# bridgedp/hunter_bipedal_control

Measured on AMD Instinct MI355X. Metric: MPC+WBC updates/sec (batch=4096, N=100, 12-DoF), higher is better.
Workload: dtype f64; 1 GPU; 4096 distinct hunter instances (4096/GPU, state seed 1234 + id), trot gait from t = 0.1, cmd_vel (0.3, 0, 0, 0), N=100 shooting intervals (dt 0.015 s), node tables generated on the device (hb_refgen_update, per-knot IK joint references), 1 SQP iteration + WeightedWbc per update, x0 of every call perturbed by measurement noise (sigma 0.01) so that no call re-solves a converged problem: every line s; batch_per_gpu=4096, total_instances=4096, horizon_nodes=100

## Files before the change

### hunter_bipedal_control_amd/csrc/hb_lq.hpp

```cpp
#pragma once
#include "hb_model.hpp"
#include "hb_tile.hpp"

namespace hb {

struct DevConfig {
  double Q_diag[HB_NX];
  double R_FF_diag[12];
  double R_jj[HB_NJ * HB_NJ];
  double friction_mu, friction_reg, friction_gripper, friction_shift, fb_mu, fb_delta;
  double soft_w;
  double pos_b[2], vel_b[2], force_b[2], force_lim[2];
  double kp_normal, zv_gain, zv_off, xy_gain;
  double g_max, g_min, alpha_decay, alpha_min, gamma_c, armijo, delta_tol;
  double torque_limits[5];
  double wbc_mu, swing_kp, swing_kd, bh_kp, bh_kd, ba_kp, ba_kd, w_swing, w_base, w_force, wbc_eps;
  int wbc_max_iter, wbc_type;
  double default_joint_state[HB_NJ];
  int debug_stop;
  int wbc_reg_steps;
  int wbc_eps_mode;
};

constexpr int NU_T = 12;
// ... 417 lines not shown
      const int s_n = c_slot(i, 0), s_x = c_slot(i, 1);
      CDt[r * 12 + s_n] = cf[i] ? v[3 * i + 2] : v[3 * i];
      CDt[r * 12 + s_x] = cf[i] ? v[3 * i] : v[3 * i + 1];
      CDt[r * 12 + s_x + 1] = cf[i] ? v[3 * i + 1] : v[3 * i + 2];
    }
  }
  {
    const double inv_m = rcp_t(M.total_mass);
    WaveTile<2, 1> tl;
    tile_init(cx, tl, 29, 9, [J2](int r, int c) {
      const double v = J2[((r >= 19 ? r : 19) - 10) * 9 + c];
      return r >= 19 ? v : 0.0;
    });
    tile_mma<8, 9, false, 9, false, 6>(cx, tl, J1, J2 + 27, 29, 9);
    tile_store_pre(cx, tl, 29, 9, [J1, J2](int r, int c) { return J1[r * 9 + c] + J2[r * 9 + c]; },
                   [ABt, dt](int r, int c, double acc, double j12) {
                     const int dir = j_dir(r), i = j_frow(c);
                     ABt[dir * 12 + i] = (dir == i ? 1.0 : 0.0) + 0.5 * dt * j12 + 0.5 * dt * dt * acc;
                   });
    for (int idx = cx.lane; idx < 108 + 132 + 27; idx += cx.nlanes) {
      if (idx < 108) {
        const int fd = idx / 9, c = idx - 9 * fd, j = fd / 3, a = fd - 3 * j;
        double g1[3], g2[3];
#pragma unroll
        for (int pt = 0; pt < 2; ++pt) {
          const double* fr_in = lds + LqLds::fr_slot(pt, j);
          const double rx = fr_in[0], ry = fr_in[1], rz = fr_in[2];
          double* g = pt == 0 ? g1 : g2;
          g[0] = (a == 1 ? -rz : (a == 2 ? ry : 0.0)) * inv_m;
          g[1] = (a == 0 ? rz : (a == 2 ? -rx : 0.0)) * inv_m;
          g[2] = (a == 0 ? -ry : (a == 1 ? rx : 0.0)) * inv_m;
        }
        double acc = inv_m * J2[a * 9 + c];
#pragma unroll
        for (int k = 0; k < 3; ++k) acc += J2[(3 + k) * 9 + c] * g1[k];
        const double lin = c < 3 ? g1[c] + g2[c] : 0.0;
        ABt[(22 + fd) * 12 + j_frow(c)] = 0.5 * dt * lin + 0.5 * dt * dt * acc;
      } else if (idx < 240) {
        const int e = idx - 108, dir = e / 3, i = e - 3 * dir;
        const bool force_i = dir >= 22 && dir < 34 && (dir - 22) % 3 == i;
        ABt[dir * 12 + i] = (dir == i ? 1.0 : 0.0) + (force_i ? dt * inv_m : 0.0);
      } else {
        const int e = idx - 240, dir = 6 + e / 9, i = 3 + e % 9;
        ABt[dir * 12 + i] = dir == i ? 1.0 : 0.0;
      }
    }
  }
  for (int i = cx.lane; i < 22; i += cx.nlanes)
    xplus[i] = (i < 12) ? xs[i] + 0.5 * dt * (fv[i] + xplus[i]) : xs[i] + dt * us[i];
  cx.sync();
#if defined(__HIP_DEVICE_COMPILE__)
  if (cx.lane < 22) { lds[LqLds::park + cx.lane] = xref_reg; lds[LqLds::xnext_park + cx.lane] = xnext_reg; }
#endif
  HB_ABLATE_STOP(C.debug_stop == form::LQ_COMPOSE);
  int n_f = 0;
  for (int i = 0; i < HB_NC; ++i)
    if (cf[i]) n_f += 3;

  {
    WaveTile<1, 2> tg;
    tile_init(cx, tg, 10, 32, [](int, int) { return 0.0; });
    tile_mma<12, 12, false, 12, true>(cx, tg, CDt + 22 * 12, CDt, 10, 32, [cfm](int slot) { return slot_is_eq(slot, cfm) ? 1.0 : 0.0; },
                                      EqStepLive{cfm});
    tile_store(cx, tg, 10, 32, [W, GtG](int k, int r, double v) {
      double* dst = r < 22 ? W + k * 23 + r : GtG + k * 10 + r - 22;
      *dst = v;
    });
  }
  for (int k = cx.lane; k < 10; k += cx.nlanes) {
    double s = 0;
#pragma unroll
    for (int slot = 0; slot < 12; ++slot) {
      const double w = slot_is_eq(slot, cfm) ? 1.0 : 0.0;
      s += (w * CDt[(22 + k) * 12 + slot]) * rowval[slot];
    }
    W[k * 23 + 22] = s;
  }
  cx.sync();
  double* Lc = Kx;
  double* col = Kx + 100;
  double* Linv = Kx + 112;
  int rank_l = 0, donemask = 0;
  int ei0 = 0, ej0 = cx.lane;
  while (ej0 > ei0) { ej0 -= ei0 + 1; ++ei0; }
#if defined(__HIP_DEVICE_COMPILE__)
  {
    static_assert(Ctx::nlanes == 64, "one triangle element per lane");
    const bool own = cx.lane < 55;
    const bool diag = own && ei0 == ej0;
    double g = own ? GtG[ei0 * 10 + ej0] : 0.0;
    const double tol = 1e-10 * wave_max_pos_f64(diag ? g : 0.0);
    for (int i = cx.lane; i < 124; i += cx.nlanes) Kx[i] = 0.0;
    cx.sync();
    for (int st = 0; st < 10; ++st) {
      const double v = (diag && !((donemask >> ei0) & 1)) ? g : -1.0;
      const double best = wave_max_pos_f64(v);
      if (!(best > tol)) break;
      const unsigned long long hit = __ballot(v == best);
      const int ps = __builtin_amdgcn_readlane(ei0, __ffsll(hit) - 1);
      const double rinv = rsqrt_t(best), lss = best * rinv;
      if (own && (ei0 == ps || ej0 == ps)) {
        const int k = (ei0 == ps) ? ej0 : ei0;
        if (!((donemask >> k) & 1)) {
          const double l = (k == ps) ? lss : g * rinv;
          col[k] = l;
          Lc[st * 10 + k] = l;
        }
      }
      if (cx.lane == 0) { perm[st] = ps; Linv[st] = rinv; }
      cx.sync();
      donemask |= 1 << ps;
      if (own && !((donemask >> ei0) & 1) && !((donemask >> ej0) & 1)) g -= col[ei0] * col[ej0];
      cx.sync();
      rank_l = st + 1;
    }
  }
#else
  double tol;
  {
    double dmax0 = 0;
    for (int i = 0; i < 10; ++i) dmax0 = fmax(dmax0, GtG[i * 10 + i]);
    tol = 1e-10 * dmax0;
  }
  for (int i = cx.lane; i < 124; i += cx.nlanes) Kx[i] = 0.0;
  cx.sync();
  for (int st = 0; st < 10; ++st) {
    int ps = -1;
    double best = -1.0;
    for (int i = 0; i < 10; ++i) {
      const double dv = GtG[i * 11];
      if (!((donemask >> i) & 1) && dv > best) { best = dv; ps = i; }
    }
    if (!(best > tol)) break;
    const double rinv = rsqrt_t(best), lss = best * rinv;
    for (int k = cx.lane; k < 10; k += cx.nlanes) {
      if (!((donemask >> k) & 1)) {
        const double l = (k == ps) ? lss : GtG[(k > ps ? k * 10 + ps : ps * 10 + k)] * rinv;
        col[k] = l;
        Lc[st * 10 + k] = l;
      }
    }
    if (cx.lane == 0) { perm[st] = ps; Linv[st] = rinv; }
    cx.sync();
    donemask |= 1 << ps;
    for (int e = cx.lane; e < 55; e += cx.nlanes) {
      int i = ei0, j = ej0;
      if (e != cx.lane) { i = 0; j = e; while (j > i) { j -= i + 1; ++i; } }
      if (!((donemask >> i) & 1) && !((donemask >> j) & 1)) GtG[i * 10 + j] -= col[i] * col[j];
    }
    cx.sync();
    rank_l = st + 1;
  }
#endif
  if (cx.lane == 0) {
    int w = rank_l;
    for (int i = 0; i < 10; ++i)
      if (!((donemask >> i) & 1)) perm[w++] = i;
  }
  cx.sync();
  HB_ABLATE_STOP(C.debug_stop == form::LQ_FACTOR);
  const int rank = rank_l;
  const int nz = 10 - rank;
  {
    double Lr[45], dinv[10];
    int pm[10];
#pragma unroll
    for (int a = 0; a < 10; ++a) { pm[a] = perm[a]; dinv[a] = Linv[a]; }
#pragma unroll
    for (int a = 1; a < 10; ++a) {
#pragma unroll
      for (int t = 0; t < a; ++t) Lr[a * (a - 1) / 2 + t] = Lc[t * 10 + pm[a]];
    }
    cx.sync();
    auto write_col = [Kx, Z, &pm, rank](int c, bool zlive, int pf, const double* y) {
      if (c < 23) {
#pragma unroll
        for (int a = 0; a < 10; ++a) Kx[pm[a] * LqLds::LDK + c] = y[a];
      } else {
#pragma unroll
        for (int a = 0; a < 10; ++a) Z[pm[a] * LqLds::LDK + c - 23] = zlive ? (a < rank ? -y[a] : (pm[a] == pf ? 1.0 : 0.0)) : 0.0;
      }
    };
#if !defined(__HIP_DEVICE_COMPILE__)
    double ycols[29][10];
    bool ylive[29];
    int ypf[29];
#endif
    for (int cc = cx.lane; cc < 29; cc += cx.nlanes) {
      const int c = 28 - cc;
      const bool isz = c >= 23;
      const int bz = c - 23;
      const bool zlive = isz && bz < nz;
      const int pf = zlive ? perm[rank + bz] : 0;
      double y[10];
#pragma unroll
      for (int a = 0; a < 10; ++a) {
        double sacc = -W[pm[a] * 23 + (isz ? 0 : c)];
#pragma unroll
        for (int t = 0; t < a; ++t) sacc -= Lr[a * (a - 1) / 2 + t] * y[t];
        y[a] = sacc * dinv[a];
      }
      if (isz) {
#pragma unroll
        for (int a = 0; a < 10; ++a) y[a] = zlive ? Lc[a * 10 + pf] : 0.0;
      }
#pragma unroll
      for (int a = 9; a >= 0; --a) {
        double sacc = y[a];
#pragma unroll
        for (int t = a + 1; t < 10; ++t) sacc -= Lr[t * (t - 1) / 2 + a] * y[t];
        y[a] = sacc * dinv[a];
      }
#if defined(__HIP_DEVICE_COMPILE__)
      write_col(c, zlive, pf, y);
#else
      for (int a = 0; a < 10; ++a) ycols[c][a] = y[a];
      ylive[c] = zlive;
      ypf[c] = pf;
#endif
    }
#if !defined(__HIP_DEVICE_COMPILE__)
    cx.sync();
    for (int cc = cx.lane; cc < 29; cc += cx.nlanes) write_col(cc, ylive[cc], ypf[cc], ycols[cc]);
#endif
  }

  HB_ABLATE_STOP(C.debug_stop == form::LQ_SOLVES);
#if defined(__HIP_DEVICE_COMPILE__)
  double cw_reg = 0.0, clo_reg = 0.0, chi_reg = 0.0;
  double rj0_reg = 0.0, rj1_reg = 0.0;
  if (in.consts) {
    rj0_reg = C.R_jj[cx.lane];
    if (cx.lane < 36) rj1_reg = C.R_jj[64 + cx.lane];
    __builtin_amdgcn_sched_barrier(0);
  }
  if (!in.consts) {
    const int role = cx.lane;
    if (role < 22) {
      cw_reg = C.Q_diag[role];
      if (role >= 12) { clo_reg = M.q_lower[role - 12]; chi_reg = M.q_upper[role - 12]; }
    } else if (role < 34) {
      cw_reg = C.R_FF_diag[role - 22];
    } else if (role < 44) {
      clo_reg = M.qd_limit[role - 34];
    }
  }
#endif
  for (int i = cx.lane; i < 22; i += cx.nlanes) xplus[i] -= xnext_at(i);
  cx.sync();
  const int ntil = n_f + nz;
  int flist = 0;
  {
    int cnt = 0;
    for (int i = 0; i < HB_NC; ++i)
      if (cf[i]) { flist |= i << (2 * cnt); ++cnt; }
  }
  double* btmp = lds + LqLds::btmp;
  {
    WaveTile<1, 2> ta;
    tile_init(cx, ta, 12, 22, [ABt](int row, int c) { return ABt[c * 12 + row]; });
    tile_mma<12, 12, true, LDK, false, 10>(cx, ta, ABt + 34 * 12, Kx, 12, LDK);
#if defined(__HIP_DEVICE_COMPILE__)
    if (in.consts) {
      W[cx.lane] = rj0_reg;
      if (cx.lane < 36) W[64 + cx.lane] = rj1_reg;
      __builtin_amdgcn_sched_barrier(0);
    }
#endif
    tile_store_rm_cols<REC_LD>(cx, ta, 12, 0, 22, rec + rec_A(0, 0));
    tile_store_rm_cols<1>(cx, ta, 12, 22, 23, btmp - 22);
    tile_store_rm_cols<REC_LD>(cx, ta, 12, 23, 23 + nz, rec + rec_A(0, 0) + n_f);
  }
  for (int c = cx.lane; c < 22; c += cx.nlanes) {
#pragma unroll
    for (int j = 0; j < 10; ++j) {
      const double kx = Kx[j * LDK + c];
      rec[rec_A(12 + j, c)] = (c == 12 + j ? 1.0 : 0.0) + dt * kx;
      rec[REC_KX + j * 22 + c] = kx;
    }
  }
  cx.sync();
  HB_ABLATE_STOP(C.debug_stop == form::LQ_DEFECT);
  for (int row = cx.lane; row < 22; row += cx.nlanes) {
#pragma unroll
    for (int col = 0; col < NU_T; ++col) {
      if (col < n_f) {
        const int foot = (flist >> (2 * (col / 3))) & 3;
        rec[rec_B(row, col)] = row < 12 ? ABt[(22 + 3 * foot + col % 3) * 12 + row] : 0.0;
      } else if (col >= ntil) {
        rec[rec_B(row, col)] = 0.0;
      } else if (row >= 12) {
        rec[rec_B(row, col)] = dt * Z[(row - 12) * LDK + col - n_f];
      }
    }
    double s = xplus[row];
    if (row >= 12) rec[REC_DQ + row - 12] = s;
    if (row < 12) {
      s += btmp[row];
      for (int i = 0; i < HB_NC; ++i)
        if (!cf[i])
          for (int a = 0; a < 3; ++a) s -= ABt[(22 + 3 * i + a) * 12 + row] * us[3 * i + a];
    } else {
      s += dt * Kx[(row - 12) * LDK + 22];
    }
    rec[rec_b(row)] = s;
  }
  HB_ABLATE_STOP(C.debug_stop == form::LQ_B_COLUMNS);
  double* red = Mm;
  {
    int nc = 0;
    for (int i = 0; i < HB_NC; ++i) nc += cf[i];
    const double fz_nom = nc > 0 ? M.total_mass * M.gravity / nc : 0.0;
    const RelaxedBarrierD fb{C.fb_mu, C.fb_delta};
    const RelaxedBarrierD bp{C.pos_b[0], C.pos_b[1]}, bv{C.vel_b[0], C.vel_b[1]}, bf{C.force_b[0], C.force_b[1]};
    auto cone = [&](int i, double& h, double* g, double& H00, double& H01, double& H11) {
      const double Fx = us[3 * i], Fy = us[3 * i + 1], Fz = us[3 * i + 2];
      const double t2 = Fx * Fx + Fy * Fy + C.friction_reg, tn = sqrt(t2), t32 = tn * t2;
      h = C.friction_mu * (Fz + C.friction_gripper) - tn;
      const double itn = rcp_t(tn), it32 = rcp_t(t32);
      g[0] = -Fx * itn; g[1] = -Fy * itn; g[2] = C.friction_mu;
      H00 = -(Fy * Fy + C.friction_reg) * it32; H01 = Fx * Fy * it32; H11 = -(Fx * Fx + C.friction_reg) * it32;
    };
    double* coneb = Rjj;
    for (int i = cx.lane; i < HB_NC; i += cx.nlanes) {
      double h = 1.0, g[3] = {0.0, 0.0, 0.0}, H00 = 0.0, H01 = 0.0, H11 = 0.0, pv = 0.0, p1 = 0.0, p2 = 0.0;
      if (cf[i]) {
        cone(i, h, g, H00, H01, H11);
        pv = fb.value(h); p1 = fb.d1(h); p2 = fb.d2(h);
      }
      double* cb = coneb + 12 * i;
      cb[0] = h; cb[1] = g[0]; cb[2] = g[1]; cb[3] = g[2]; cb[4] = H00; cb[5] = H01; cb[6] = H11; cb[7] = pv; cb[8] = p1; cb[9] = p2;
    }
    cx.sync();
    double shift_sum = 0;
    for (int i = 0; i < HB_NC; ++i)
      if (cf[i]) shift_sum += -coneb[12 * i + 8] * C.friction_shift;
#if defined(__HIP_DEVICE_COMPILE__)
    double rff_reg[3] = {0.0, 0.0, 0.0};
    const double* Rc_lds = C.R_jj;
    if (in.consts) {
      const int l = cx.lane, foot = (l - 56) & 3;
      const double g1 = wave_gather_f64(in.c_tab, l < 22 ? l + 22 : (l < 44 ? l + 20 : 22 + 3 * foot));
      const double g2 = wave_gather_f64(in.c_tab, l < 22 ? l + 32 : 23 + 3 * foot);
      const double g3 = wave_gather_f64(in.c_tab, 24 + 3 * foot);
      cw_reg = in.c_tab;
      clo_reg = g1;
      chi_reg = g2;
      rff_reg[0] = g1; rff_reg[1] = g2; rff_reg[2] = g3;
      Rc_lds = W;
    }
#endif
    for (int role = cx.lane; role < 64; role += cx.nlanes) {
      double pc = 0, pd = 0, pe = 0;
      double bval = 0.0, bd1 = 0.0, bd2 = 0.0;
      {
        bool hasb = false;
        double h1 = 1.0, h2 = 1.0, bmu = 0.0, bdel = 1.0;
        if (role >= 12 && role < 22) {
          const int j = role - 12;
          const double h = xs[role];
#if defined(__HIP_DEVICE_COMPILE__)
          (void)j;
          hasb = true; h1 = h - clo_reg; h2 = chi_reg - h; bmu = bp.mu; bdel = bp.delta;
#else
          hasb = true; h1 = h - M.q_lower[j]; h2 = M.q_upper[j] - h; bmu = bp.mu; bdel = bp.delta;
#endif
        } else if (role >= 22 && role < 34) {
          const int m = role - 22;
          if (m - 3 * (m / 3) == 2) {
            const double h = us[m];
            hasb = true; h1 = h - C.force_lim[0]; h2 = C.force_lim[1] - h; bmu = bf.mu; bdel = bf.delta;
          }
        } else if (role >= 34 && role < 44) {
          const int k = role - 34;
#if defined(__HIP_DEVICE_COMPILE__)
          const double hv = us[12 + k], vl = clo_reg;
#else
          const double hv = us[12 + k], vl = M.qd_limit[k];
#endif
          hasb = true; h1 = hv + vl; h2 = vl - hv; bmu = bv.mu; bdel = bv.delta;
        }
        if (hasb) {
          const RelaxedBarrierD rb{bmu, bdel};
          bval = rb.value(h1) + rb.value(h2);
          bd1 = rb.d1(h1) - rb.d1(h2);
          bd2 = rb.d2(h1) + rb.d2(h2);
        }
      }
      if (role < 22) {
        const int i = role;
        const double dxv = xs[i] - xref_at(i);
#if defined(__HIP_DEVICE_COMPILE__)
        const double Qi = cw_reg;
#else
        const double Qi = C.Q_diag[i];
#endif
        double qd_ = Qi + shift_sum, qg = Qi * dxv;
        pc += 0.5 * Qi * dxv * dxv;
        if (i >= 12) {
          pc += bval;
          qg += bd1;
          qd_ += bd2;
        }
        Qd[i] = qd_;
        qx[i] = qg;
        const double dd = xplus[i];
        pd += dd * dd;
      } else if (role < 34) {
        const int m = role - 22, foot = m / 3, a = m % 3;
        const double du = us[m] - ((a == 2 && cf[foot]) ? fz_nom : 0.0);
#if defined(__HIP_DEVICE_COMPILE__)
        const double Rm_ = cw_reg;
#else
        const double Rm_ = C.R_FF_diag[m];
#endif
        double rg = Rm_ * du;
        pc += 0.5 * Rm_ * du * du;
        if (cf[foot]) {
          rg += coneb[12 * foot + 8] * coneb[12 * foot + 1 + a];
        } else {
          pe += us[m] * us[m];
        }
        if (a == 2) {
          pc += bval;
          rg += bd1;
        }
        ru[m] = rg;
      } else if (role < 44) {
        const int k = role - 34;
        double sacc = 0;
#if defined(__HIP_DEVICE_COMPILE__)
        for (int l = 0; l < HB_NJ; ++l) sacc += Rc_lds[k * 10 + l] * us[12 + l];
#else
        for (int l = 0; l < HB_NJ; ++l) sacc += C.R_jj[k * 10 + l] * us[12 + l];
#endif
        pc += 0.5 * us[12 + k] * sacc;
        pc += bval;
        ru[12 + k] = sacc + bd1;
        scal[4 + k] = bd2 + shift_sum;
      } else if (role < 56) {
        const int sl = role - 44;
        const double rv = rowval[sl];
        if (slot_is_eq(sl, cfm)) pe += rv * rv;
        else pc += 0.5 * C.soft_w * rv * rv;
      } else if (role < 60) {
        const int foot = role - 56;
        double blk[9];
        for (int e = 0; e < 9; ++e) blk[e] = 0.0;
#if defined(__HIP_DEVICE_COMPILE__)
        for (int a = 0; a < 3; ++a) blk[4 * a] = (in.consts ? rff_reg[a] : C.R_FF_diag[3 * foot + a]) + shift_sum;
#else
        for (int a = 0; a < 3; ++a) blk[4 * a] = C.R_FF_diag[3 * foot + a] + shift_sum;
#endif
        {
          const double h = us[3 * foot + 2];
          blk[8] += bf.d2(h - C.force_lim[0]) + bf.d2(C.force_lim[1] - h);
        }
        if (cf[foot]) {
          const double* cb = coneb + 12 * foot;
          const double g[3] = {cb[1], cb[2], cb[3]}, H00 = cb[4], H01 = cb[5], H11 = cb[6];
          const double p1 = cb[8], p2 = cb[9];
          pc += cb[7];
          for (int a = 0; a < 3; ++a)
            for (int bb = 0; bb < 3; ++bb) blk[3 * a + bb] += p2 * g[a] * g[bb];
          blk[0] += p1 * H00; blk[1] += p1 * H01; blk[3] += p1 * H01; blk[4] += p1 * H11;
        }
        for (int e = 0; e < 9; ++e) RFF[9 * foot + e] = blk[e];
      }
#if defined(__HIP_DEVICE_COMPILE__)
      pc = wave_sum_f64(pc);
      pd = wave_sum_f64(pd);
      pe = wave_sum_f64(pe);
      if (role == 0) { scal[0] = pc; scal[1] = pd; scal[2] = pe; }
#else
      red[role] = pc;
      red[64 + role] = pd;
      red[128 + role] = pe;
#endif
    }
  }
  cx.sync();
#if !defined(__HIP_DEVICE_COMPILE__)
  for (int w = cx.lane; w < 3; w += cx.nlanes) {
    double sacc = 0;
    for (int l = 0; l < 64; ++l) sacc += red[64 * w + l];
    scal[w] = sacc;
  }
  cx.sync();
#endif
  HB_ABLATE_STOP(C.debug_stop == form::LQ_COST);
  for (int c = cx.lane; c < 32; c += cx.nlanes) {
    double s = 0;
#pragma unroll
    for (int slot = 0; slot < 8; ++slot) {
      const double w = slot_is_soft(slot, cfm) ? 1.0 : 0.0;
      s += (w * rowval[slot]) * CDt[c * 12 + slot];
    }
    if (c < 22) qx[c] += C.soft_w * s;
    else ru[12 + c - 22] += C.soft_w * s;
  }
  {
    const double sw = C.soft_w;
#if defined(__HIP_DEVICE_COMPILE__)
    const double* Rc = in.consts ? W : C.R_jj;
#else
    const double* Rc = C.R_jj;
#endif
    WaveTile<1, 2> tg;
    tile_init(cx, tg, 10, 32, [Rc, scal](int k, int r) {
      const int rr = (r >= 22 ? r : 22) - 22;
      const double v = Rc[k * 10 + rr], sc = scal[4 + k];
      return r >= 22 ? v + (rr == k ? sc : 0.0) : 0.0;
    });
    tile_mma<12, 12, false, 12, true>(cx, tg, CDt + 22 * 12, CDt, 10, 32, [cfm, sw](int slot) { return slot_is_soft(slot, cfm) ? sw : 0.0; },
                                      SoftStepLive{cfm});
    tile_store(cx, tg, 10, 32, [Pj, Rjj](int k, int r, double v) {
      double* dst = r < 22 ? Pj + k * 22 + r : Rjj + k * 10 + r - 22;
      *dst = v;
    });
  }
  cx.sync();
  {
    WaveTile<1, 2> tm;
    tile_init(cx, tm, 10, 23, [Pj, ru](int k, int c) {
      const double a = Pj[k * 22 + (c < 22 ? c : 21)], b = ru[12 + k];
      return c < 22 ? a : b;
    });
    tile_mma<12, 10, false, LDK, false, 10>(cx, tm, Rjj, Kx, 10, LDK);
    tile_store_rm<LDK>(cx, tm, 10, LDK, Mm);
  }
  cx.sync();

  HB_ABLATE_STOP(C.debug_stop == form::LQ_SOFT_ROWS);
  {
    const double sw = C.soft_w;
    auto soft = [cfm, sw](int slot) { return slot_is_soft(slot, cfm) ? sw : 0.0; };
    const SoftStepLive soft_live{cfm};
    WaveTile<1, 2> t0;
    WaveTile<1, 1> t1;
    tile_init(cx, t0, 16, 22, [Qd](int a, int b) { const double d = Qd[a]; return a == b ? d : 0.0; });
    tile_init(cx, t1, 6, 6, [Qd](int a, int b) { const double d = Qd[16 + a]; return a == b ? d : 0.0; });
    tile_mma<12, 12, false, 12, true>(cx, t0, CDt, CDt, 16, 22, soft, soft_live);
    tile_mma<12, 12, false, 12, true>(cx, t1, CDt + 16 * 12, CDt + 16 * 12, 6, 6, soft, soft_live);
    tile_set_col(cx, t0, 22, 16, [qx](int a) { return qx[a]; });
    tile_set_col(cx, t1, 6, 6, [qx](int a) { return qx[16 + a]; });
    tile_mma<12, LDK, true, LDK, false, 10>(cx, t0, Kx, Mm, 16, 23);
    tile_mma<12, LDK, true, LDK, false, 10>(cx, t1, Kx + 16, Mm + 16, 6, 7);
    tile_mma<12, 22, true, LDK, false, 10>(cx, t0, Pj, Kx, 16, 23);
    tile_mma<12, 22, true, LDK, false, 10>(cx, t1, Pj + 16, Kx + 16, 6, 7);
    tile_store(cx, t0, 16, 23, [rec, dt](int a, int b, double v) {
      double* dst = b < 22 ? rec + REC_QT + rec_Qidx(a, b) : rec + REC_qT + a;
      if (a <= b) *dst = dt * v;
    });
    tile_store(cx, t1, 6, 7, [rec, dt](int a, int b, double v) {
      double* dst = b < 6 ? rec + REC_QT + rec_Qidx(16 + a, 16 + b) : rec + REC_qT + 16 + a;
      if (a <= b) *dst = dt * v;
    });
  }
  HB_ABLATE_STOP(C.debug_stop == form::LQ_Q);
  for (int a = cx.lane; a < 22; a += cx.nlanes) {
    rec[REC_QF + a] = dt * qx[a];
    rec[REC_RF + a] = dt * ru[a];
  }
  if (nz > 0) {
    WaveTile<1, 2> tp;
    tile_init(cx, tp, 6, 22, [](int, int) { return 0.0; });
    tile_mma<12, LDK, true, LDK, false, 10>(cx, tp, Z, Mm, 6, LDK);
    tile_store_rm_cols<REC_LD>(cx, tp, nz, 0, 23, rec + rec_P(n_f, 0), dt);
    tile_store_rm_cols<REC_LD>(cx, tp, nz, 23, 23 + nz, rec + rec_P(n_f, 0) + n_f, dt);
  }
  for (int c = cx.lane; c < 22; c += cx.nlanes) {
#pragma unroll
    for (int a = 0; a < NU_T; ++a)
      if (a < n_f || a >= ntil) rec[rec_P(a, c)] = 0.0;
  }
  HB_ABLATE_STOP(C.debug_stop == form::LQ_P);
  for (int idx = cx.lane; idx < NU_T * NU_T; idx += cx.nlanes) {
    const int ca = idx / NU_T, cb = idx % NU_T;
    double s = 0.0;
    bool pad_diag = false;
    if (ca < n_f && cb < n_f) {
      if (ca / 3 == cb / 3) {
        const int foot = (flist >> (2 * (ca / 3))) & 3;
        s = RFF[9 * foot + 3 * (ca % 3) + (cb % 3)];
      }
    } else if (ca >= n_f && ca < ntil && cb >= n_f && cb < ntil) {
      continue;
    } else if (ca >= ntil && ca == cb) {
      pad_diag = true;
    }
    rec[rec_R(ca, cb)] = pad_diag ? 1.0 : dt * s;
  }
  for (int col = cx.lane; col < NU_T; col += cx.nlanes) {
    double s = 0.0;
    if (col < n_f) {
      const int foot = (flist >> (2 * (col / 3))) & 3;
      s = ru[3 * foot + col % 3];
    } else if (col < ntil) {
      continue;
    }
    rec[rec_r(col)] = dt * s;
  }
  HB_ABLATE_STOP(C.debug_stop == form::LQ_R);
  for (int k = cx.lane; k < 10; k += cx.nlanes) rec[REC_KE + k] = Kx[k * LDK + 22];
  for (int idx = cx.lane; idx < 60; idx += cx.nlanes) rec[REC_Z + idx] = idx % 6 < nz ? Z[(idx / 6) * LDK + idx % 6] : 0.0;
  for (int i = cx.lane; i < 12; i += cx.nlanes) rec[REC_DF + i] = cf[i / 3] ? 0.0 : -us[i];
  if (cx.lane == 0) {
    rec[REC_META + 0] = double(n_f);
    rec[REC_META + 1] = double(nz);
    rec[REC_META + 2] = double(in.mode);
    rec[REC_META + 3] = dt * scal[0];
    rec[REC_META + 4] = dt * scal[1];
    rec[REC_META + 5] = dt * scal[2];
    rec[REC_DT] = dt;
  }
}

template <class Ctx, class XR, class XN>
HB_HD void lq_node_dense(const Ctx& cx, const DevModel& M, const DevConfig& C, const NodeIn& in, double* lds, double* rec, XR xref_at, XN xnext_at) {
  const LqP1 P1 = lq_p1(lds);
  for (int task = cx.lane; task < 58; task += cx.nlanes) lq_tangent_task(M, C, lds, in.mode, task >= 29 ? 1 : 0, task >= 29 ? task - 29 : task);
  cx.sync();
#if defined(__HIP_DEVICE_COMPILE__)
  if (cx.lane < 24) {
    const int pt = cx.lane / 12, e = cx.lane - 12 * pt;
    lds[LqLds::fr_slot(pt, e / 3) + e % 3] = (P1.CDt + 6 * 12)[cx.lane];
  }
  cx.sync();
#endif
  HB_ABLATE_STOP(C.debug_stop == form::LQ_DIRECTIONS);
  for (int task = cx.lane; task < 3; task += cx.nlanes) lq_closed_task(C, lds, in.mode, task);
  cx.sync();
  lq_tail(cx, M, C, in, lds, rec, xref_at, xnext_at);
}

struct LqPark {
  static constexpr int per_lane = 256, size = 4 * per_lane;
  static constexpr int n_feet = LEGJ_FEET, n_vj = 206, n_row = 212, n_fr0 = 215, n_ns0 = 218, n_rm0 = 227, n_fr1 = 232, n_ns1 = 235, n_rm1 = 244, n_end = 249;
  static constexpr int trip_max = 16;
  static constexpr int n_tab0 = 192;
  static constexpr int stash_pt = 39 * trip_max;
  static constexpr int sncs = 0, feet = 512, jc_tab = 896;
  static constexpr int hand = 0;
  static constexpr int ns_dest(int pt, int j) {
    if (j < 6) return LqLds::fv + 12 + 6 * pt + j;
    if (j < 18) return (pt == 0 ? LqLds::fv : LqLds::xe) + (j - 6);
    if (j < 33) return LqLds::LV + pt * LqLds::LVP + (j - 18);
    return LqLds::xe + 12 + 3 * pt + (j - 33);
  }
  static constexpr int dest(int n, int e) {
    if (n < n_vj) return (n < n_feet && n % LEGJ_STRIDE == LEGJ_MS && n >= n_tab0) ? -1 : LqLds::LJ + e * LEGJ_SIZE + n;
    if (n < n_row) return LqLds::LV + (e >> 1) * LqLds::LVP + 15 + 6 * (e & 1) + (n - n_vj);
    if (n < n_fr0) return LqLds::rowval + 3 * e + (n - n_row);
    if (n < n_ns0) return LqLds::CDt + 72 + 3 * e + (n - n_fr0);
    if (n < n_rm0) return ns_dest(0, 9 * e + (n - n_ns0));
    if (n < n_fr1) return (e >> 1) == 0 ? LqLds::LJ + e * LEGJ_SIZE + (n - n_rm0) * LEGJ_STRIDE + LEGJ_MS : -1;
    if (n < n_ns1) return LqLds::CDt + 72 + 12 + 3 * e + (n - n_fr1);
    if (n < n_rm1) return ns_dest(1, 9 * e + (n - n_ns1));
    if (n < n_end) return (e >> 1) == 1 ? LqLds::LJ + e * LEGJ_SIZE + (n - n_rm1) * LEGJ_STRIDE + LEGJ_MS : -1;
    return -1;
  }
};
struct LqParkTab { int d[LqPark::per_lane - LqPark::n_tab0][4]; };
constexpr LqParkTab lq_park_tab() {
  LqParkTab t{};
  for (int n = LqPark::n_tab0; n < LqPark::per_lane; ++n)
    for (int e = 0; e < 4; ++e) t.d[n - LqPark::n_tab0][e] = LqPark::dest(n, e);
  return t;
}
static_assert(LqPark::jc_tab + 160 <= LqLds::total && 2 * LqPark::stash_pt <= LqLds::total && LqPark::hand + 36 * LqPark::trip_max <= LqPark::stash_pt,
              "the value phase's LDS lives in the node's");
static_assert(LqPark::n_tab0 % 4 == 0 && LqPark::n_tab0 <= LqPark::n_feet && LqPark::n_tab0 / 4 * 8 % 64 == 0, "whole rounds of the read-back go to the leg blocks");
static_assert(LqPark::per_lane % 8 == 0 && LEGJ_STRIDE % 8 == 0 && LEGJ_FEET % 8 == 0, "entries leave eight at a time");
#if defined(__HIP_DEVICE_COMPILE__)
static_assert(LqLds::SC == LqLds::fv + 12, "the sin / cos pairs sit in the second half of fv");
__device__ const LqParkTab kLqParkTab = lq_park_tab();
struct LqTrip {
  double* lds;
  double* park;
  int tlen, nt, lane;
  int dbg;
};
#if defined(HB_ABLATE) && defined(HB_LQV_TRACE)
#define HB_LQV_MARK(tr, i) if ((tr).dbg == form::LQT_TRACE && blockIdx.x == 1000 && (tr).lane == 0) reinterpret_cast<long long*>((tr).lds + LqLds::total - 24)[i] = __builtin_readcyclecounter();
#else
#define HB_LQV_MARK(tr, i)
#endif
__device__ __forceinline__ void lq_wave_order() {
  __builtin_amdgcn_fence(__ATOMIC_ACQ_REL, "wavefront");
  __builtin_amdgcn_wave_barrier();
}
__device__ __forceinline__ void lq_park_out(const LqTrip& tr, int n0, const double* v8) {
  typedef double d2 __attribute__((ext_vector_type(2)));
  int lane = tr.lane;
  asm volatile("" : "+v"(lane));
  lane &= 63;
  const int t = lane >> 2, e = lane & 3;
  if (t < tr.nt && !(HB_ABLATE_ON && tr.dbg == form::LQT_PARK_NOTHING)) {
    double* line = tr.park + (size_t(n0 >> 2) * tr.tlen + t) * 16 + 2 * e;
#pragma unroll
    for (int i = 0; i < 8; i += 2) {
      d2 x;
      x.x = v8[i]; x.y = v8[i + 1];
      *reinterpret_cast<d2*>(line + (size_t(i >> 2) * tr.tlen * 16) + ((i & 3) >> 1) * 8) = x;
    }
  }
}
__device__ __forceinline__ void lq_trip_stage_constants(const DevModel& M, double* lds, int lane) {
  for (int i = lane; i < 160; i += 64) {
    const int j = i >> 4, c = i & 15, b = j + 1;
    lds[LqPark::jc_tab + i] = c < 3 ? M.axis[j][c] : (c < 6 ? M.origin[j][c - 3] : (c < 9 ? M.com[b][c - 6] : (c < 15 ? M.inertia[b][c - 9] : M.mass[b])));
  }
}
__device__ __forceinline__ void lq_trip_leg_pass(const LqTrip& tr, const DevModel& M, int leg, double dts, const double* xk, const double* uk, double* val) {
  const double* jct = tr.lds + LqPark::jc_tab + leg * 80;
  double* sncs = tr.lds + LqPark::sncs + 8 * tr.lane - 2;
  double* pfl = tr.lds + LqPark::feet + 6 * tr.lane;
  const int j0 = 5 * leg;
  double qa[5], qr[5];
#pragma unroll
  for (int k = 0; k < 5; ++k) { qr[k] = uk[12 + j0 + k]; qa[k] = xk[12 + j0 + k] + dts * qr[k]; }
  auto pick = [](const double* v, int k) { return k == 0 ? v[0] : (k == 1 ? v[1] : (k == 2 ? v[2] : (k == 3 ? v[3] : v[4]))); };
  Mat3<double> R = Mat3<double>::identity();
  Vec3<double> op, om, w;
  HB_LQV_MARK(tr, 1)
#pragma unroll 1
  for (int k = 0; k < 5; ++k) {
    const double* jc = jct + 16 * k;
    const double ax[3] = {jc[0], jc[1], jc[2]};
    const Vec3<double> o = op + R * Vec3<double>(jc[3], jc[4], jc[5]);
    const Vec3<double> a = R * Vec3<double>(ax[0], ax[1], ax[2]);
    const double qd = pick(qr, k);
    om = om + qd * a;
    w = w + qd * cross(a, o);
    double sk, ck;
    sincos_bounded(pick(qa, k), sk, ck);
    if (k > 0) { sncs[2 * k] = sk; sncs[2 * k + 1] = ck; }
    R = R * axis_rot_sc<double>(ax, sk, ck);
    op = o;
  }
  if (HB_ABLATE_ON && tr.dbg == form::LQT_VALUES_FWD) return;
  HB_LQV_MARK(tr, 2)
#pragma unroll
  for (int f = 0; f < 2; ++f) {
    const int ci = leg + 2 * f;
    st3(pfl + 3 * f, op + R * Vec3<double>(M.contact_offset[ci][0], M.contact_offset[ci][1], M.contact_offset[ci][2]));
  }
  double ms = 0.0;
  Vec3<double> mc, lin, ang, vj[2];
  Sym3<double> IO;
#pragma unroll 1
  for (int k = 4; k >= 0; --k) {
    const double* jc = jct + 16 * k;
    const double ax[3] = {jc[0], jc[1], jc[2]};
    const Vec3<double> o = op;
    const Vec3<double> a = R * Vec3<double>(ax[0], ax[1], ax[2]);
    const double mb = jc[15];
    const Vec3<double> c = o + R * Vec3<double>(jc[6], jc[7], jc[8]);
    const double in[6] = {jc[9], jc[10], jc[11], jc[12], jc[13], jc[14]};
    ms += mb;
    mc = mc + mb * c;
    IO = IO + (rotate_inertia<double>(R, in) + point_inertia<double>(mb, c));
    const Vec3<double> l = cross(a, mc - ms * o);
    const Vec3<double> L = IO * a - cross(mc, cross(a, o));
    const double qd = pick(qr, k);
    lin = lin + qd * l;
// ... 320 lines not shown
```

### hunter_bipedal_control_amd/csrc/hb_math.hpp

```cpp
#pragma once
#include <math.h>

#if defined(__HIPCC__)
#include <hip/hip_runtime.h>
#define HB_HD __host__ __device__ __forceinline__
#else
#define HB_HD inline
#endif

#include "hb_forms.hpp"

#if defined(HB_ABLATE)
#define HB_ABLATE_STOP(cond) do { if (cond) return; } while (0)
#define HB_ABLATE_ON 1
#else
#if defined(__HIP_DEVICE_COMPILE__)
#if defined(HB_PHASE_MARK)
#define HB_PHASE_STR2(x) #x
#define HB_PHASE_STR(x) HB_PHASE_STR2(x)
#define HB_ABLATE_STOP(cond) asm volatile("; HB_PHASE line " HB_PHASE_STR(__LINE__) ::: "memory")
#else
#define HB_ABLATE_STOP(cond) asm volatile("" ::: "memory")
#endif
#else
#define HB_ABLATE_STOP(cond) do { } while (0)
#endif
#define HB_ABLATE_ON 0
#endif

namespace hb {

struct Dual1 {
  double v, d;
  HB_HD Dual1() : v(0.0), d(0.0) {}
  HB_HD Dual1(double a) : v(a), d(0.0) {}
  HB_HD Dual1(double a, double b) : v(a), d(b) {}
};
HB_HD Dual1 operator+(Dual1 a, Dual1 b) { return {a.v + b.v, a.d + b.d}; }
HB_HD Dual1 operator-(Dual1 a, Dual1 b) { return {a.v - b.v, a.d - b.d}; }
HB_HD Dual1 operator-(Dual1 a) { return {-a.v, -a.d}; }
HB_HD Dual1 operator*(Dual1 a, Dual1 b) { return {a.v * b.v, fma(a.v, b.d, a.d * b.v)}; }
HB_HD double rcp_t(double a) {
#if defined(__HIP_DEVICE_COMPILE__)
  double r = __builtin_amdgcn_rcp(a);
  r = fma(fma(-a, r, 1.0), r, r);
  r = fma(fma(-a, r, 1.0), r, r);
  return r;
#else
  return 1.0 / a;
#endif
}
HB_HD Dual1 operator/(Dual1 a, Dual1 b) {
  const double inv = rcp_t(b.v), q = a.v * inv;
  return {q, (a.d - q * b.d) * inv};
}
HB_HD Dual1 rcp_t(Dual1 a) {
  const double r = rcp_t(a.v);
  return {r, -a.d * r * r};
}
HB_HD Dual1 operator*(double a, Dual1 b) { return {a * b.v, a * b.d}; }
HB_HD Dual1 operator*(Dual1 b, double a) { return {a * b.v, a * b.d}; }
HB_HD Dual1 operator+(Dual1 a, double b) { return {a.v + b, a.d}; }
HB_HD Dual1 operator-(Dual1 a, double b) { return {a.v - b, a.d}; }
HB_HD Dual1 operator-(double a, Dual1 b) { return {a - b.v, -b.d}; }
HB_HD Dual1& operator+=(Dual1& a, Dual1 b) { a.v += b.v; a.d += b.d; return a; }
HB_HD Dual1& operator-=(Dual1& a, Dual1 b) { a.v -= b.v; a.d -= b.d; return a; }
HB_HD void sincos_reduced(double a, double& s, double& c);
HB_HD void sincos_t(double a, double& s, double& c) {
  if (!(fabs(a) < 1.0e5)) { s = sin(a); c = cos(a); return; }
  sincos_reduced(a, s, c);
}
HB_HD void sincos_bounded(double a, double& s, double& c) {
  double sv, cv;
  sincos_reduced(fabs(a) < 1.0e5 ? a : 0.0, sv, cv);
  const bool ok = fabs(a) < 1.0e5;
  s = ok ? sv : NAN;
  c = ok ? cv : NAN;
}
HB_HD void sincos_reduced(double a, double& s, double& c) {
  const double k = rint(a * 6.36619772367581382433e-01);
  double r = fma(-k, 1.57079632673412561417e+00, a);
  r = fma(-k, 6.07710050630396597660e-11, r);
  r = fma(-k, 2.02226624871116645580e-21, r);
  r = fma(-k, 8.47842766036889956997e-32, r);
  const double z = r * r;
  double ps = fma(z, 1.58969099521155010221e-10, -2.50507602534068634195e-08);
  ps = fma(z, ps, 2.75573137070700676789e-06);
  ps = fma(z, ps, -1.98412698298579493134e-04);
  ps = fma(z, ps, 8.33333333332248946124e-03);
  ps = fma(z, ps, -1.66666666666666324348e-01);
  const double sr = fma(z * r, ps, r);
  double pc = fma(z, -1.13596475577881948265e-11, 2.08757232129817482790e-09);
  pc = fma(z, pc, -2.75573143513906633035e-07);
  pc = fma(z, pc, 2.48015872894767294178e-05);
  pc = fma(z, pc, -1.38888888888741095749e-03);
  pc = fma(z, pc, 4.16666666666666019037e-02);
  const double cr = fma(z * z, pc, fma(-0.5, z, 1.0));
  const int q = int(k) & 3;
  const double s0 = (q & 1) ? cr : sr, c0 = (q & 1) ? sr : cr;
  s = (q & 2) ? -s0 : s0;
  c = ((q + 1) & 2) ? -c0 : c0;
}
HB_HD void sincos_t(Dual1 a, Dual1& s, Dual1& c) {
  double sv, cv;
  sincos_t(a.v, sv, cv);
  s = {sv, cv * a.d};
  c = {cv, -sv * a.d};
}
HB_HD double log_fd(double x) {
  int k;
#if defined(__HIP_DEVICE_COMPILE__)
  double m = __builtin_amdgcn_frexp_mant(x);
  k = __builtin_amdgcn_frexp_exp(x);
#else
  double m = frexp(x, &k);
#endif
  if (m < 0.70710678118654752440) { m *= 2.0; k -= 1; }
  const double f = m - 1.0;
  const double s = f * rcp_t(2.0 + f);
  const double z = s * s, w = z * z;
  const double t1 = w * fma(w, fma(w, 1.531383769920937332e-01, 2.222219843214978396e-01), 3.999999999940941908e-01);
  const double t2 = z * fma(w, fma(w, fma(w, 1.479819860511658591e-01, 1.818357216161805012e-01), 2.857142874366239149e-01),
                            6.666666666666735130e-01);
  const double R = t2 + t1, hfsq = 0.5 * f * f, dk = double(k);
  return dk * 6.93147180369123816490e-01 - ((hfsq - fma(s, hfsq + R, dk * 1.90821492927058770002e-10)) - f);
}
HB_HD double log_t(double x) {
#if defined(__HIP_DEVICE_COMPILE__)
  return log_fd(x);
#else
  return log(x);
#endif
}
HB_HD void sincos_known(double sv, double cv, double, double& s, double& c) { s = sv; c = cv; }
HB_HD void sincos_known(double sv, double cv, Dual1 a, Dual1& s, Dual1& c) {
  s = {sv, cv * a.d};
  c = {cv, -sv * a.d};
}
#if defined(__HIP_DEVICE_COMPILE__)
template <int CTRL>
__device__ __forceinline__ double dpp_full_f64(double v) {
  const int lo_ = __builtin_amdgcn_mov_dpp(__double2loint(v), CTRL, 0xf, 0xf, true);
  const int hi_ = __builtin_amdgcn_mov_dpp(__double2hiint(v), CTRL, 0xf, 0xf, true);
  return __hiloint2double(hi_, lo_);
}
template <int CTRL, int BANK>
__device__ __forceinline__ double dpp_carry_f64(double v, double& carrier) {
  const int lo_ = __builtin_amdgcn_update_dpp(__double2loint(carrier), __double2loint(v), CTRL, 0xf, BANK, true);
  const int hi_ = __builtin_amdgcn_update_dpp(__double2hiint(carrier), __double2hiint(v), CTRL, 0xf, BANK, true);
  carrier = __hiloint2double(hi_, lo_);
  return carrier;
}
__device__ __forceinline__ double wave_max_f64(double v) {
#define HB_DPP_MAX(ctrl, rmask)                                                              \
  {                                                                                          \
    const int lo_ = __double2loint(v), hi_ = __double2hiint(v);                              \
    const int lo2_ = __builtin_amdgcn_update_dpp(lo_, lo_, ctrl, rmask, 0xf, false);         \
    const int hi2_ = __builtin_amdgcn_update_dpp(hi_, hi_, ctrl, rmask, 0xf, false);         \
    v = fmax(v, __hiloint2double(hi2_, lo2_));                                               \
  }
  HB_DPP_MAX(0x111, 0xf)
  HB_DPP_MAX(0x112, 0xf)
  HB_DPP_MAX(0x114, 0xf)
  HB_DPP_MAX(0x118, 0xf)
  HB_DPP_MAX(0x142, 0xa)
  HB_DPP_MAX(0x143, 0xc)
#undef HB_DPP_MAX
  return __hiloint2double(__builtin_amdgcn_readlane(__double2hiint(v), 63), __builtin_amdgcn_readlane(__double2loint(v), 63));
}
__device__ __forceinline__ double wave_max_pos_f64(double v) {
#define HB_DPP_MAX0(ctrl, rmask)                                                                            \
  {                                                                                                         \
    const int lo2_ = __builtin_amdgcn_update_dpp(0, __double2loint(v), ctrl, rmask, 0xf, true);             \
    const int hi2_ = __builtin_amdgcn_update_dpp(0, __double2hiint(v), ctrl, rmask, 0xf, true);             \
    const double o_ = __hiloint2double(hi2_, lo2_);                                                         \
    asm("v_max_f64 %0, %1, %2" : "=v"(v) : "v"(v), "v"(o_));                                                \
  }
#define HB_DPP_MAXF(ctrl)                                                                                   \
  {                                                                                                         \
    const double o_ = dpp_full_f64<ctrl>(v);                                                                \
    asm("v_max_f64 %0, %1, %2" : "=v"(v) : "v"(v), "v"(o_));                                                \
  }
  HB_DPP_MAXF(0x111)
// ... 256 lines not shown
```

Baseline: 546,100 updates/s.

## Parallelize LQ record emission and batch loads ahead of stores

Rewrites several serial or branchy stages of the LQ node record emission. The permutation fill now runs across lanes using popcount, and Z is merged into the Kx buffer writes. The B, P, R, r, KE, Z and DF writes are restructured so that all operands are loaded first and pinned with asm barriers, P padding rows are zeroed with two-wide vector stores, and lane work is spread evenly. The aim is to remove lane-0 serialization and interleaved load/store latency in this phase, at the cost of more complex index logic that risks correctness errors (for example, Z is no longer written separately, which other readers may depend on).

```diff
diff --git a/hunter_bipedal_control_amd/csrc/hb_lq.hpp b/hunter_bipedal_control_amd/csrc/hb_lq.hpp
--- a/hunter_bipedal_control_amd/csrc/hb_lq.hpp
+++ b/hunter_bipedal_control_amd/csrc/hb_lq.hpp
@@ -593,10 +593,9 @@
     rank_l = st + 1;
   }
 #endif
-  if (cx.lane == 0) {
-    int w = rank_l;
-    for (int i = 0; i < 10; ++i)
-      if (!((donemask >> i) & 1)) perm[w++] = i;
+  for (int i = cx.lane; i < 10; i += cx.nlanes) {
+    const unsigned fr = ~unsigned(donemask) & 0x3ffu;
+    if ((fr >> i) & 1) perm[rank_l + __builtin_popcount(fr & ((1u << i) - 1u))] = i;
   }
   cx.sync();
   HB_ABLATE_STOP(C.debug_stop == form::LQ_FACTOR);
@@ -613,13 +612,12 @@
       for (int t = 0; t < a; ++t) Lr[a * (a - 1) / 2 + t] = Lc[t * 10 + pm[a]];
     }
     cx.sync();
-    auto write_col = [Kx, Z, &pm, rank](int c, bool zlive, int pf, const double* y) {
-      if (c < 23) {
-#pragma unroll
-        for (int a = 0; a < 10; ++a) Kx[pm[a] * LqLds::LDK + c] = y[a];
-      } else {
-#pragma unroll
-        for (int a = 0; a < 10; ++a) Z[pm[a] * LqLds::LDK + c - 23] = zlive ? (a < rank ? -y[a] : (pm[a] == pf ? 1.0 : 0.0)) : 0.0;
+    auto write_col = [Kx, &pm, rank](int c, bool zlive, int pf, const double* y) {
+      const bool isz = c >= 23;
+#pragma unroll
+      for (int a = 0; a < 10; ++a) {
+        const double zv = zlive ? (a < rank ? -y[a] : (pm[a] == pf ? 1.0 : 0.0)) : 0.0;
+        Kx[pm[a] * LqLds::LDK + c] = isz ? zv : y[a];
       }
     };
 #if !defined(__HIP_DEVICE_COMPILE__)
@@ -723,28 +721,54 @@
   cx.sync();
   HB_ABLATE_STOP(C.debug_stop == form::LQ_DEFECT);
   for (int row = cx.lane; row < 22; row += cx.nlanes) {
-#pragma unroll
-    for (int col = 0; col < NU_T; ++col) {
-      if (col < n_f) {
-        const int foot = (flist >> (2 * (col / 3))) & 3;
-        rec[rec_B(row, col)] = row < 12 ? ABt[(22 + 3 * foot + col % 3) * 12 + row] : 0.0;
-      } else if (col >= ntil) {
-        rec[rec_B(row, col)] = 0.0;
-      } else if (row >= 12) {
-        rec[rec_B(row, col)] = dt * Z[(row - 12) * LDK + col - n_f];
-      }
-    }
-    double s = xplus[row];
-    if (row >= 12) rec[REC_DQ + row - 12] = s;
-    if (row < 12) {
-      s += btmp[row];
+    const bool mom = row < 12;
+    const int rm = mom ? row : 0, rj = mom ? 0 : row - 12;
+    double bf[HB_NC][3], uf[HB_NC][3], zc[6];
+#pragma unroll
+    for (int i = 0; i < HB_NC; ++i)
+#pragma unroll
+      for (int a = 0; a < 3; ++a) { bf[i][a] = ABt[(22 + 3 * i + a) * 12 + rm]; uf[i][a] = us[3 * i + a]; }
+#pragma unroll
+    for (int b = 0; b < 6; ++b) zc[b] = Z[rj * LDK + b];
+    double defect = xplus[row], bt = btmp[rm], ke = Kx[rj * LDK + 22];
+#pragma unroll
+    for (int i = 0; i < HB_NC; ++i)
+#pragma unroll
+      for (int a = 0; a < 3; ++a) { keep_here(bf[i][a]); keep_here(uf[i][a]); }
+#pragma unroll
+    for (int b = 0; b < 6; ++b) keep_here(zc[b]);
+    keep_here(defect); keep_here(bt); keep_here(ke);
+    double* brow = rec + rec_B(row, 0);
+    {
+      double* bcol = brow;
+#pragma unroll
       for (int i = 0; i < HB_NC; ++i)
-        if (!cf[i])
-          for (int a = 0; a < 3; ++a) s -= ABt[(22 + 3 * i + a) * 12 + row] * us[3 * i + a];
-    } else {
-      s += dt * Kx[(row - 12) * LDK + 22];
-    }
-    rec[rec_b(row)] = s;
+        if (cf[i]) {
+#pragma unroll
+          for (int a = 0; a < 3; ++a) bcol[a] = mom ? bf[i][a] : 0.0;
+          bcol += 3;
+        }
+    }
+    if (!mom) {
+      double* bcol = brow + n_f;
+      const int nzc = nz < NU_T - n_f ? nz : NU_T - n_f;
+#pragma unroll
+      for (int b = 0; b < 6; ++b)
+        if (b < nzc) bcol[b] = dt * zc[b];
+      for (int b = 6; b < nzc; ++b) bcol[b] = dt * Z[rj * LDK + b];
+    }
+#pragma unroll
+    for (int col = 6; col < NU_T; ++col)
+      if (col >= ntil) brow[col] = 0.0;
+    if (!mom) rec[REC_DQ + rj] = defect;
+    double s = defect + bt;
+#pragma unroll
+    for (int i = 0; i < HB_NC; ++i)
+      if (!cf[i]) {
+#pragma unroll
+        for (int a = 0; a < 3; ++a) s -= bf[i][a] * uf[i][a];
+      }
+    rec[rec_b(row)] = mom ? s : defect + dt * ke;
   }
   HB_ABLATE_STOP(C.debug_stop == form::LQ_B_COLUMNS);
   double* red = Mm;
@@ -1010,49 +1034,57 @@
     tile_store_rm_cols<REC_LD>(cx, tp, nz, 0, 23, rec + rec_P(n_f, 0), dt);
     tile_store_rm_cols<REC_LD>(cx, tp, nz, 23, 23 + nz, rec + rec_P(n_f, 0) + n_f, dt);
   }
-  for (int c = cx.lane; c < 22; c += cx.nlanes) {
-#pragma unroll
-    for (int a = 0; a < NU_T; ++a)
-      if (a < n_f || a >= ntil) rec[rec_P(a, c)] = 0.0;
+  const int n_zero = n_f + (ntil < NU_T ? NU_T - ntil : 0);
+  for (int idx = cx.lane; idx < 3 * 64; idx += cx.nlanes) {
+    const int z = idx >> 4, pr = idx & 15;
+    if (z < n_zero && pr < 11) store_zero2(rec + rec_P(z < n_f ? z : z + nz, 2 * pr));
   }
   HB_ABLATE_STOP(C.debug_stop == form::LQ_P);
-  for (int idx = cx.lane; idx < NU_T * NU_T; idx += cx.nlanes) {
-    const int ca = idx / NU_T, cb = idx % NU_T;
-    double s = 0.0;
-    bool pad_diag = false;
-    if (ca < n_f && cb < n_f) {
-      if (ca / 3 == cb / 3) {
-        const int foot = (flist >> (2 * (ca / 3))) & 3;
-        s = RFF[9 * foot + 3 * (ca % 3) + (cb % 3)];
-      }
-    } else if (ca >= n_f && ca < ntil && cb >= n_f && cb < ntil) {
-      continue;
-    } else if (ca >= ntil && ca == cb) {
-      pad_diag = true;
-    }
-    rec[rec_R(ca, cb)] = pad_diag ? 1.0 : dt * s;
-  }
-  for (int col = cx.lane; col < NU_T; col += cx.nlanes) {
-    double s = 0.0;
-    if (col < n_f) {
-      const int foot = (flist >> (2 * (col / 3))) & 3;
-      s = ru[3 * foot + col % 3];
-    } else if (col < ntil) {
-      continue;
-    }
-    rec[rec_r(col)] = dt * s;
+  for (int idx = cx.lane; idx < 64; idx += cx.nlanes) {
+    static_assert(LqLds::ru > LqLds::RFF, "one base for both operands");
+    const int lk = idx >> 4, e = idx & 15, cb = e - 1, lr = lk < 3 ? lk : 0;
+    const bool live = e <= NU_T;
+    const double dz = dt * 0.0;
+    double op[HB_NC];
+#pragma unroll
+    for (int j = 0; j < HB_NC; ++j) {
+      const int foot = (flist >> (2 * j)) & 3, cr = cb - 3 * j;
+      op[j] = RFF[e == 0 ? (LqLds::ru - LqLds::RFF) + 3 * foot + lr : 9 * foot + 3 * lr + (cr >= 0 && cr < 3 ? cr : 0)];
+    }
+#pragma unroll
+    for (int j = 0; j < HB_NC; ++j) keep_here(op[j]);
+    double* rf = rec + rec_r(lk) + e;
+#pragma unroll
+    for (int j = 0; j < HB_NC; ++j)
+      if (3 * j < n_f) {
+        const int cr = cb - 3 * j;
+        if (live && lk < 3) rf[3 * j * REC_LD] = dt * ((e == 0 || (cr >= 0 && cr < 3)) ? op[j] : 0.0);
+      }
+    double* rk = rec + rec_r(n_f + lk) + e;
+#pragma unroll
+    for (int q = 0; q < 3; ++q)
+      if (n_f + 4 * q < NU_T) {
+        const int ca = n_f + 4 * q + lk;
+        const bool kern_row = ca < ntil;
+        if (live && ca < NU_T && !(kern_row && (e == 0 || (cb >= n_f && cb < ntil)))) rk[4 * q * REC_LD] = (!kern_row && cb == ca) ? 1.0 : dz;
+      }
   }
   HB_ABLATE_STOP(C.debug_stop == form::LQ_R);
-  for (int k = cx.lane; k < 10; k += cx.nlanes) rec[REC_KE + k] = Kx[k * LDK + 22];
-  for (int idx = cx.lane; idx < 60; idx += cx.nlanes) rec[REC_Z + idx] = idx % 6 < nz ? Z[(idx / 6) * LDK + idx % 6] : 0.0;
-  for (int i = cx.lane; i < 12; i += cx.nlanes) rec[REC_DF + i] = cf[i / 3] ? 0.0 : -us[i];
-  if (cx.lane == 0) {
+  for (int l = cx.lane; l < 64; l += cx.nlanes) {
+    double kev = Kx[(l < 10 ? l : 0) * LDK + 22], zv = Z[(l < 60 ? l / 6 : 0) * LDK + l % 6], uv = us[l < 12 ? l : 0];
+    double c0 = scal[0], c1 = scal[1], c2 = scal[2];
+    keep_here(kev); keep_here(zv); keep_here(uv); keep_here(c0); keep_here(c1); keep_here(c2);
+    double* rl = rec + REC_KE + l;
+    if (l < 10) rl[0] = kev;
+    if (l < 60) rl[REC_Z - REC_KE] = l % 6 < nz ? zv : 0.0;
+    if (l < 12) rl[REC_DF - REC_KE] = ((cfm >> (l / 3)) & 1) ? 0.0 : -uv;
+    if (l != 0) continue;
     rec[REC_META + 0] = double(n_f);
     rec[REC_META + 1] = double(nz);
     rec[REC_META + 2] = double(in.mode);
-    rec[REC_META + 3] = dt * scal[0];
-    rec[REC_META + 4] = dt * scal[1];
-    rec[REC_META + 5] = dt * scal[2];
+    rec[REC_META + 3] = dt * c0;
+    rec[REC_META + 4] = dt * c1;
+    rec[REC_META + 5] = dt * c2;
     rec[REC_DT] = dt;
   }
 }
diff --git a/hunter_bipedal_control_amd/csrc/hb_math.hpp b/hunter_bipedal_control_amd/csrc/hb_math.hpp
--- a/hunter_bipedal_control_amd/csrc/hb_math.hpp
+++ b/hunter_bipedal_control_amd/csrc/hb_math.hpp
@@ -29,6 +29,22 @@
 #endif
 
 namespace hb {
+
+HB_HD void keep_here(double& v) {
+#if defined(__HIP_DEVICE_COMPILE__)
+  asm volatile("" : "+v"(v));
+#else
+  (void)v;
+#endif
+}
+HB_HD void store_zero2(double* p) {
+#if defined(__HIP_DEVICE_COMPILE__)
+  typedef double d2 __attribute__((ext_vector_type(2)));
+  *reinterpret_cast<d2*>(p) = d2{0.0, 0.0};
+#else
+  p[0] = 0.0; p[1] = 0.0;
+#endif
+}
 
 struct Dual1 {
   double v, d;
```

Measured after the change: 551,500 updates/s, median of 2. No clear change (+1.0%).
